# nv-dvl/nerfmatch

Measured on AMD Instinct MI355X. Metric: rays*samples/sec, higher is better.
Workload: dtype fp16x3 (fp16 MFMA on hi/lo-split fp32 operands, three products per fp32 product, fp32 accumulate; fp32 everywhere else)

## Files before the change

nerfmatch_amd/csrc/nerf_fwd_bf16.hip:

```cpp
#include "nerf_split_chain.h"

namespace {
using namespace nmbf;
using nmsample::HALF_PI_F32, nmsample::SCAN_TILE, nmsample::frustum, nmsample::ray_consts, nmsample::lift_var, nmsample::ipe_fast, nmsample::view_row_value;
using nmsample::alpha_of, nmsample::trans_factor, nmsample::sigmoid, nmsample::scan_before_barrier, nmsample::scan_after_barrier, nmsample::scan_carry;
using nmsample::first_max;
static_assert(TILE == SCAN_TILE, "the compositing scan of nerf_sample.h spans two wavefronts");

template <int PART, bool OWN>
__device__ __forceinline__ void tap_prefetch(Ctx& cx) {
  if constexpr (PART == 0) __builtin_amdgcn_s_barrier();
  const char* src = reinterpret_cast<const char*>(cx.tapw);
#pragma unroll
  for (int q = (PART == 0 ? 0 : 4); q < (PART == 0 ? 4 : 7); ++q) {
    const char* sp = src + q * 4096;
    const float* dp = q < 4 ? cx.tap_ring + q * 1024 : cx.tap_ipe + (q - 4) * 1024;
    const unsigned lds = (unsigned)__builtin_amdgcn_readfirstlane((int)(unsigned)(size_t)(const __attribute__((address_space(3))) float*)dp);
    if constexpr (OWN) {
      asm volatile("s_mov_b32 m0, %0\n\tglobal_load_lds_dwordx4 %1, off\n\tglobal_load_lds_dwordx4 %1, off offset:1024\n\t"
                   "global_load_lds_dwordx4 %1, off offset:2048\n\tglobal_load_lds_dwordx4 %1, off offset:3072"
                   :: "s"(lds), "v"(sp) : "memory");
      continue;
    }
    unsigned m0_saved;
    asm volatile("s_mov_b32 %0, m0\n\ts_mov_b32 m0, %1\n\tglobal_load_lds_dwordx4 %2, off\n\tglobal_load_lds_dwordx4 %2, off offset:1024\n\t"
                 "global_load_lds_dwordx4 %2, off offset:2048\n\tglobal_load_lds_dwordx4 %2, off offset:3072\n\ts_mov_b32 m0, %0"
                 : "=&s"(m0_saved) : "s"(lds), "v"(sp) : "memory");
  }
}

__device__ __forceinline__ void dpp_pairs8(float (&o)[8], const float (&x)[8], const float (&y)[8], bool eight) {
  if (eight)
    asm("s_nop 1\n"
        "v_add_f32_dpp %0, %8, %8 row_mirror row_mask:0xf bank_mask:0x3\n\tv_add_f32_dpp %1, %9, %9 row_mirror row_mask:0xf bank_mask:0x3\n\t"
        "v_add_f32_dpp %2, %10, %10 row_mirror row_mask:0xf bank_mask:0x3\n\tv_add_f32_dpp %3, %11, %11 row_mirror row_mask:0xf bank_mask:0x3\n\t"
        "v_add_f32_dpp %4, %12, %12 row_mirror row_mask:0xf bank_mask:0x3\n\tv_add_f32_dpp %5, %13, %13 row_mirror row_mask:0xf bank_mask:0x3\n\t"
        "v_add_f32_dpp %6, %14, %14 row_mirror row_mask:0xf bank_mask:0x3\n\tv_add_f32_dpp %7, %15, %15 row_mirror row_mask:0xf bank_mask:0x3\n\t"
        "v_add_f32_dpp %0, %16, %16 row_mirror row_mask:0xf bank_mask:0xc\n\tv_add_f32_dpp %1, %17, %17 row_mirror row_mask:0xf bank_mask:0xc\n\t"
        "v_add_f32_dpp %2, %18, %18 row_mirror row_mask:0xf bank_mask:0xc\n\tv_add_f32_dpp %3, %19, %19 row_mirror row_mask:0xf bank_mask:0xc\n\t"
        "v_add_f32_dpp %4, %20, %20 row_mirror row_mask:0xf bank_mask:0xc\n\tv_add_f32_dpp %5, %21, %21 row_mirror row_mask:0xf bank_mask:0xc\n\t"
        "v_add_f32_dpp %6, %22, %22 row_mirror row_mask:0xf bank_mask:0xc\n\tv_add_f32_dpp %7, %23, %23 row_mirror row_mask:0xf bank_mask:0xc"
        : "=&v"(o[0]), "=&v"(o[1]), "=&v"(o[2]), "=&v"(o[3]), "=&v"(o[4]), "=&v"(o[5]), "=&v"(o[6]), "=&v"(o[7])
        : "v"(x[0]), "v"(x[1]), "v"(x[2]), "v"(x[3]), "v"(x[4]), "v"(x[5]), "v"(x[6]), "v"(x[7]),
          "v"(y[0]), "v"(y[1]), "v"(y[2]), "v"(y[3]), "v"(y[4]), "v"(y[5]), "v"(y[6]), "v"(y[7]));
  else
    asm("s_nop 1\n"
        "v_add_f32_dpp %0, %8, %8 row_half_mirror row_mask:0xf bank_mask:0x5\n\tv_add_f32_dpp %1, %9, %9 row_half_mirror row_mask:0xf bank_mask:0x5\n\t"
        "v_add_f32_dpp %2, %10, %10 row_half_mirror row_mask:0xf bank_mask:0x5\n\tv_add_f32_dpp %3, %11, %11 row_half_mirror row_mask:0xf bank_mask:0x5\n\t"
        "v_add_f32_dpp %4, %12, %12 row_half_mirror row_mask:0xf bank_mask:0x5\n\tv_add_f32_dpp %5, %13, %13 row_half_mirror row_mask:0xf bank_mask:0x5\n\t"
        "v_add_f32_dpp %6, %14, %14 row_half_mirror row_mask:0xf bank_mask:0x5\n\tv_add_f32_dpp %7, %15, %15 row_half_mirror row_mask:0xf bank_mask:0x5\n\t"
        "v_add_f32_dpp %0, %16, %16 row_half_mirror row_mask:0xf bank_mask:0xa\n\tv_add_f32_dpp %1, %17, %17 row_half_mirror row_mask:0xf bank_mask:0xa\n\t"
        "v_add_f32_dpp %2, %18, %18 row_half_mirror row_mask:0xf bank_mask:0xa\n\tv_add_f32_dpp %3, %19, %19 row_half_mirror row_mask:0xf bank_mask:0xa\n\t"
        "v_add_f32_dpp %4, %20, %20 row_half_mirror row_mask:0xf bank_mask:0xa\n\tv_add_f32_dpp %5, %21, %21 row_half_mirror row_mask:0xf bank_mask:0xa\n\t"
        "v_add_f32_dpp %6, %22, %22 row_half_mirror row_mask:0xf bank_mask:0xa\n\tv_add_f32_dpp %7, %23, %23 row_half_mirror row_mask:0xf bank_mask:0xa"
        : "=&v"(o[0]), "=&v"(o[1]), "=&v"(o[2]), "=&v"(o[3]), "=&v"(o[4]), "=&v"(o[5]), "=&v"(o[6]), "=&v"(o[7])
        : "v"(x[0]), "v"(x[1]), "v"(x[2]), "v"(x[3]), "v"(x[4]), "v"(x[5]), "v"(x[6]), "v"(x[7]),
          "v"(y[0]), "v"(y[1]), "v"(y[2]), "v"(y[3]), "v"(y[4]), "v"(y[5]), "v"(y[6]), "v"(y[7]));
}
template <int XOR>
__device__ __forceinline__ void quad_add8(float (&v)[8]) {
  if (XOR == 1)
    asm("s_nop 1\n"
        "v_add_f32_dpp %0, %0, %0 quad_perm:[1,0,3,2] row_mask:0xf bank_mask:0xf\n\tv_add_f32_dpp %1, %1, %1 quad_perm:[1,0,3,2] row_mask:0xf bank_mask:0xf\n\t"
        "v_add_f32_dpp %2, %2, %2 quad_perm:[1,0,3,2] row_mask:0xf bank_mask:0xf\n\tv_add_f32_dpp %3, %3, %3 quad_perm:[1,0,3,2] row_mask:0xf bank_mask:0xf\n\t"
        "v_add_f32_dpp %4, %4, %4 quad_perm:[1,0,3,2] row_mask:0xf bank_mask:0xf\n\tv_add_f32_dpp %5, %5, %5 quad_perm:[1,0,3,2] row_mask:0xf bank_mask:0xf\n\t"
        "v_add_f32_dpp %6, %6, %6 quad_perm:[1,0,3,2] row_mask:0xf bank_mask:0xf\n\tv_add_f32_dpp %7, %7, %7 quad_perm:[1,0,3,2] row_mask:0xf bank_mask:0xf"
        : "+v"(v[0]), "+v"(v[1]), "+v"(v[2]), "+v"(v[3]), "+v"(v[4]), "+v"(v[5]), "+v"(v[6]), "+v"(v[7]));
  else
    asm("s_nop 1\n"
        "v_add_f32_dpp %0, %0, %0 quad_perm:[2,3,0,1] row_mask:0xf bank_mask:0xf\n\tv_add_f32_dpp %1, %1, %1 quad_perm:[2,3,0,1] row_mask:0xf bank_mask:0xf\n\t"
        "v_add_f32_dpp %2, %2, %2 quad_perm:[2,3,0,1] row_mask:0xf bank_mask:0xf\n\tv_add_f32_dpp %3, %3, %3 quad_perm:[2,3,0,1] row_mask:0xf bank_mask:0xf\n\t"
        "v_add_f32_dpp %4, %4, %4 quad_perm:[2,3,0,1] row_mask:0xf bank_mask:0xf\n\tv_add_f32_dpp %5, %5, %5 quad_perm:[2,3,0,1] row_mask:0xf bank_mask:0xf\n\t"
        "v_add_f32_dpp %6, %6, %6 quad_perm:[2,3,0,1] row_mask:0xf bank_mask:0xf\n\tv_add_f32_dpp %7, %7, %7 quad_perm:[2,3,0,1] row_mask:0xf bank_mask:0xf"
        : "+v"(v[0]), "+v"(v[1]), "+v"(v[2]), "+v"(v[3]), "+v"(v[4]), "+v"(v[5]), "+v"(v[6]), "+v"(v[7]));
}
__device__ __forceinline__ float reduce_scatter_step16(float x, float y) {
  const auto r = __builtin_amdgcn_permlane16_swap(__float_as_uint(x), __float_as_uint(y), false, false);
  return __uint_as_float(r[0]) + __uint_as_float(r[1]);
}
__device__ __forceinline__ f32x4 reduce_scatter_16pairs(const float (&s1)[64], int lane) {
  float s2[32];
#pragma unroll
  for (int b = 0; b < 4; ++b) {
    float o[8], x[8], y[8];
#pragma unroll
    for (int i = 0; i < 8; ++i) { x[i] = s1[8 * b + i]; y[i] = s1[32 + 8 * b + i]; }
    dpp_pairs8(o, x, y, true);
#pragma unroll
    for (int i = 0; i < 8; ++i) s2[8 * b + i] = o[i];
  }
  float s3[16];
#pragma unroll
  for (int b = 0; b < 2; ++b) {
    float o[8], x[8], y[8];
#pragma unroll
    for (int i = 0; i < 8; ++i) { x[i] = s2[8 * b + i]; y[i] = s2[16 + 8 * b + i]; }
    dpp_pairs8(o, x, y, false);
#pragma unroll
    for (int i = 0; i < 8; ++i) s3[8 * b + i] = o[i];
  }
  float lo8[8], hi8[8];
#pragma unroll
  for (int i = 0; i < 8; ++i) { lo8[i] = s3[i]; hi8[i] = s3[8 + i]; }
  quad_add8<2>(lo8); quad_add8<2>(hi8);
  float s4[8];
#pragma unroll
  for (int i = 0; i < 8; ++i) s4[i] = (lane & 2) ? hi8[i] : lo8[i];
  float t8[8] = {s4[0], s4[1], s4[2], s4[3], s4[4], s4[5], s4[6], s4[7]};
  quad_add8<1>(t8);
  return (lane & 1) ? f32x4{t8[4], t8[5], t8[6], t8[7]} : f32x4{t8[0], t8[1], t8[2], t8[3]};
}
__device__ __forceinline__ f32x4 reduce_scatter_32rows(float (&v)[128], int lane) {
  float s1[64];
#pragma unroll
  for (int i = 0; i < 64; ++i) s1[i] = reduce_scatter_step16(v[i], v[64 + i]);
  return reduce_scatter_16pairs(s1, lane);
}

#define NM_MLP_DONE_WAIT() __builtin_amdgcn_s_waitcnt(0x0070)
#define NM_EPI_BARRIER() asm volatile("s_waitcnt lgkmcnt(0)\n\ts_barrier" ::: "memory")
template <int P, bool TAP7 = true>
__device__ __forceinline__ void nerf_fwd_body(const NerfArgs& a) {
  constexpr bool DENS = P == 2 && !TAP7;
  __shared__ __attribute__((aligned(16))) float sm[LDS_TOTAL];
  float* const sm_small = sm + LDS_SMALL;
  float* const ring = sm + LDS_RING;
  float* const sm_ipe = sm + LDS_IPE;
  float* const sm_sigma = sm + LDS_SCR;
  float* const sm_rgb = sm_sigma + TILE;
  float* const sm_t0 = sm_rgb + 3 * TILE;
  float* const sm_t1 = sm_t0 + TILE;
  float* const sm_mean = sm_t1 + TILE;
  float* const sm_dn = sm_mean + 3 * TILE;
  float* const sm_w = sm_dn + TILE;
  float* const sm_misc = sm_w + TILE;
  float* const sm_part = sm_misc + 32;
  float* const sm_feat = sm + LDS_FEAT;
  float* const sm_ex = sm + LDS_EX;
  int* const sm_lray = reinterpret_cast<int*>(sm + LDS_LEFT);
  float* const sm_lT = sm + LDS_LEFT + TILE;
  unsigned* const sm_rng = reinterpret_cast<unsigned*>(sm + LDS_RNG);

  const int tid = threadIdx.x, lane = tid & 63, wave = tid >> 6, s = lane & 31, hi = lane >> 5;
  const bool tail_ok = a.left && !(a.tail_viol && *a.tail_viol != 0);
  const int S = a.S, R = a.R;
  const int Sa = tail_ok ? a.Sa : S;
  const int left = tail_ok ? 1 : 0;
  const int ntiles = tail_ok ? a.ntiles : a.ntiles_full;
  const int SP = Sa < TILE ? Sa : TILE;
  const int nr = TILE / SP;
  const int nchunks = (Sa + TILE - 1) / TILE;
  const bool need_rgb = !(a.flags & NM_NERF_SKIP_RGB);
  const bool feat_max = (a.flags & NM_NERF_FEAT_MAX) != 0;
  const bool need_tap = (a.feat != nullptr) || (a.sfeat != nullptr);
  const int tap = (a.tap < 0 || a.tap > 7) ? 7 : a.tap;
  const int nslots = need_rgb ? NSLOT_FULL : NSLOT_NORGB;
  const char* const blob_slots = a.blob + (size_t)SMALL_PAD * 4;

  for (int i = tid; i < SMALL / 4; i += 256) reinterpret_cast<f32x4*>(sm_small)[i] = reinterpret_cast<const f32x4*>(a.blob)[i];
  if constexpr (P == 2) {
#pragma unroll
    for (int k = 0; k < NRANGE; ++k) sm_rng[k * 256 + tid] = 0u;
  }

  int nleft = 0;
  int bid = blockIdx.x;
#pragma unroll 1
  for (;;) {
  bool lo_pass = false;
  if (left && (nleft > TILE - 4 || (bid >= ntiles && nleft > 0))) lo_pass = true;
  else if (bid >= ntiles) break;
  const int nent = lo_pass ? nleft : 0;
  TRACE(0);
  if (need_rgb && !lo_pass && tid < nr * 48) {
    const int r2 = tid / 48, f = tid % 48;
    const int ray2 = bid * nr + r2;
    const float* rq = a.rays + (size_t)(ray2 < R ? ray2 : R - 1) * 12 + 8;
    float v = view_row_value(f, rq[f % 3], a.app_row);
    if constexpr (P == 2) {
      v *= reinterpret_cast<const float*>(a.blob)[OFF_INSCALE + (f < 27 ? 1 : 2)];
      __hip_atomic_fetch_max(sm_rng + 9 * 256 + tid, __float_as_uint(fabsf(v)), __ATOMIC_RELAXED, __HIP_MEMORY_SCOPE_WORKGROUP);
    }
    sm_ex[tid] = v;
  }
  __syncthreads();
  TRACE(1);

  const int js = wave * 32 + s;
  const int rl = js / SP;
  const int ray = lo_pass ? (js < nent ? sm_lray[js] : R) : bid * nr + rl;
  const int rc = lo_pass ? sm_lray[js < nent ? js : 0] : (ray < R ? ray : R - 1);
  const float* rp = a.rays + (size_t)rc * 12;
  const float o0 = rp[0], o1 = rp[1], o2 = rp[2], d0 = rp[3], d1 = rp[4], d2 = rp[5], radius = rp[11];
  float dsq[3], nul[3], dnorm;
  ray_consts(rp + 3, dsq, nul, dnorm);

  float red_acc = 0.f;
  float carryT = 1.f;
  float best_w = -1.f;
  float feat_run = 0.f;

  const int nch = lo_pass ? 1 : nchunks;
  for (int chunk = 0; chunk < nch; ++chunk) {
    const int sidx = lo_pass ? Sa : chunk * TILE + (js % SP);
    const float t0 = a.t[(size_t)rc * (S + 1) + sidx];
    const float t1 = a.t[(size_t)rc * (S + 1) + sidx + 1];
// ... 34 lines not shown
    if constexpr (is_split<P>()) {
      ring_open_wait<P>(cx);
    } else {
      ring_acquire<P>(blob_slots, 0, nslots, ring, wave, lane);
    }
    load_half<P>(cx.opA, ring, lane, 0);
    if constexpr (P == 1) load_half<1>(cx.opB, ring, lane, 1);
    const float* ipe_src = sm_ipe + wave * (XS * 2 * 64 * 4) + lane * 4;

    auto composite_weights = [&]() __attribute__((always_inline)) {
      const int tid2 = launder(threadIdx.x), lane2 = tid2 & 63, wave2 = tid2 >> 6;
      float alpha = 0.f, incl = 1.f;
      if (tid2 < TILE) {
        alpha = alpha_of(sm_sigma[tid2], (sm_t1[tid2] - sm_t0[tid2]) * sm_dn[tid2]);
        incl = scan_before_barrier(trans_factor(alpha), lane2, wave2, SP, sm_misc);
      }
      NM_EPI_BARRIER();
      if (tid2 < TILE) {
        const float excl = scan_after_barrier(incl, lane2, wave2, SP, sm_misc, carryT);
        sm_w[tid2] = alpha * excl;
        const int r2 = tid2 / SP, ray2 = bid * nr + r2;
        if (left && chunk == nchunks - 1 && ray2 < R && tid2 % SP == SP - 1) {
          sm_lray[nleft + r2] = ray2;
          sm_lT[nleft + r2] = excl * trans_factor(alpha);
        }
      }
      if (nchunks > 1) carryT = scan_carry(carryT, sm_misc);
    };
    auto composite_sums = [&]() __attribute__((always_inline)) {
      const int tid2 = launder(threadIdx.x);
      if (tid2 < TILE) {
        const float wgt = sm_w[tid2];
        const int r2 = tid2 / SP, ray2 = bid * nr + r2;
        if (ray2 < R) {
          const int s2 = chunk * TILE + tid2 % SP;
          a.weights[(size_t)ray2 * S + s2] = wgt;
          if (left && chunk == nchunks - 1) {
            for (int k = Sa + 1 + tid2 % SP; k < S; k += SP) a.weights[(size_t)ray2 * S + k] = 0.f;
          }
          if (a.raw && !NM_TRACE) {
            f32x4 rv = {sm_rgb[tid2], sm_rgb[TILE + tid2], sm_rgb[2 * TILE + tid2], sm_sigma[tid2]};
            *reinterpret_cast<f32x4*>(a.raw + ((size_t)ray2 * S + s2) * 4) = rv;
          }
        }
        float pq[8] = {wgt, wgt * sm_rgb[tid2], wgt * sm_rgb[TILE + tid2], wgt * sm_rgb[2 * TILE + tid2],
                       wgt * (0.5f * (sm_t0[tid2] + sm_t1[tid2])), wgt * sm_mean[tid2], wgt * sm_mean[TILE + tid2],
                       wgt * sm_mean[2 * TILE + tid2]};
        nm_half_sum_dpp8(pq);
        if ((tid2 & 31) == 16) {
          *reinterpret_cast<f32x4*>(sm_part + (tid2 >> 5) * 8) = f32x4{pq[0], pq[1], pq[2], pq[3]};
          *reinterpret_cast<f32x4*>(sm_part + (tid2 >> 5) * 8 + 4) = f32x4{pq[4], pq[5], pq[6], pq[7]};
        }
      }
    };
    auto pick_best = [&]() __attribute__((always_inline)) {
      const int tid2 = launder(threadIdx.x);
      if (tid2 < 8 * nr) {
        const int q = tid2 & 7, r2 = tid2 >> 3;
        const float* wv = sm_w + r2 * SP;
        int bi;
        const bool better = first_max(wv, SP, best_w, bi);
        if (q == 0) sm_misc[8 + r2] = better ? __int_as_float(r2 * SP + bi) : __int_as_float(-1);
        if (q >= 5 && better) red_acc = sm_mean[(q - 5) * TILE + r2 * SP + bi];
      }
    };
    auto tap7_early = [&](Ctx& c) __attribute__((always_inline)) {
      const int t2 = launder(threadIdx.x), jl = (t2 >> 6) * 32 + (t2 & 31), hl = (t2 >> 5) & 1;
      const float sigma_raw = (c.sig_part + nm_shfl_xor32(c.sig_part)) + sm_small[OFF_MISC];
      if (hl == 0) sm_sigma[jl] = sigma_raw;
      NM_EPI_BARRIER();
      composite_weights();
      NM_EPI_BARRIER();
      if (feat_max) {
        pick_best();
        NM_EPI_BARRIER();
      }
      const float desc = sm_small[OFF_DESCALE + 7];
      const float wj = sm_w[jl] * desc;
      const int best = feat_max ? __float_as_int(sm_misc[8 + jl / SP]) : -2;
      const float mult = feat_max ? (jl == best ? desc : 0.f) : wj;
      const float* bl = sm_small + OFF_BIAS + 7 * 256 + 4 * hl;
      const float s7 = sm_small[OFF_SCALE + 7];
      float s1[64];
#pragma unroll
      for (int cq = 0; cq < HS; ++cq) {
        const f32x4 b0 = *reinterpret_cast<const f32x4*>(bl + (cq >> 2) * 32 + 8 * (cq & 3));
        const f32x4 b1 = *reinterpret_cast<const f32x4*>(bl + (4 + (cq >> 2)) * 32 + 8 * (cq & 3));
#pragma unroll
        for (int e = 0; e < 4; ++e) {
          const float x = mult * __builtin_fmaxf(__builtin_fmaf(c.hv[4 * cq + e], s7, b0[e]), 0.f);
          const float y = mult * __builtin_fmaxf(__builtin_fmaf(c.hv[64 + 4 * cq + e], s7, b1[e]), 0.f);
          s1[4 * cq + e] = reduce_scatter_step16(x, y);
        }
      }
      const f32x4 sum4 = reduce_scatter_16pairs(s1, jl);
      const int r = jl & 31;
      float* prow = sm_feat + (jl >> 5) * 256 + 4 * hl;
      *reinterpret_cast<f32x4*>(prow + (r >> 2) * 32 + 16 * ((r >> 1) & 1) + 8 * (r & 1)) = sum4;
    };
    const Tap7InRegisters<decltype(tap7_early)> tap7{early, tap7_early};
    f32x16 acc[8];
    ipe_steps<P, true>(acc, cx, ipe_src);
    finish_layer<P>(acc, 0, cx);
    TRACE(3);
#pragma unroll 1
    for (int l = 1; l < 8; ++l) {
      layer_pass<P, DENS>(acc, l, cx, ipe_src, tap7);
      TRACE(3 + l);
    }
    float c_r = 0.f, c_g = 0.f, c_b = 0.f;
    if (!need_rgb) {
      if (cx.tap == 7) dump_tap(7, cx);
      NM_MLP_DONE_WAIT();
      if (cx.tap_pref) tap_prefetch<0, owns_m0<P>()>(cx);
      alpha_head(cx);
      if (cx.tap_pref) tap_prefetch<1, owns_m0<P>()>(cx);
    } else {
      const int hh = launder(lane) >> 5;
      const float* exr = sm_ex + launder(rl) * 48 + 8 * hh;
      f32x16 av[4];
      if constexpr (DENS) {
        views_hidden<P, true>(av, cx);
        dens_close(cx);
      } else views_hidden<P>(av, cx);
      fold_range<P>(cx, 7);
      bf16x8 exh[VS], exl[VS];
#pragma unroll
      for (int e = 0; e < VS; ++e) {
        float v8[8];
        if (!lo_pass) {
          const f32x4 e0 = *reinterpret_cast<const f32x4*>(exr + 16 * e), e1 = *reinterpret_cast<const f32x4*>(exr + 16 * e + 4);
          v8[0] = e0[0]; v8[1] = e0[1]; v8[2] = e0[2]; v8[3] = e0[3]; v8[4] = e1[0]; v8[5] = e1[1]; v8[6] = e1[2]; v8[7] = e1[3];
        } else {
          const float* rq = a.rays + (size_t)launder(rc) * 12 + 8;
          const float vd0 = rq[0], vd1 = rq[1], vd2 = rq[2];
#pragma unroll
          for (int i = 0; i < 8; ++i) {
            const int f = 16 * e + 8 * hh + i;
            const int ax = f % 3;
            float v = view_row_value(f, ax == 0 ? vd0 : ax == 1 ? vd1 : vd2, a.app_row);
            if constexpr (P == 2) v *= sm_small[OFF_INSCALE + (f < 27 ? 1 : 2)];
            v8[i] = v;
          }
        }
        if constexpr (is_split<P>()) split8_p<P>(v8, exh[e], exl[e]);
        else exh[e] = exl[e] = pack8_f16(v8);
      }
      views_extras<P>(av, cx, exh, exl, a.app_row == nullptr);
      TRACE(11);
      NM_MLP_DONE_WAIT();
      if (cx.tap_pref) tap_prefetch<0, owns_m0<P>()>(cx);
      const float* bv = sm_small + OFF_BVIEWS + 4 * hh;
      const float* wr = sm_small + OFF_WRGB + 4 * hh;
      float pr = 0.f, pg = 0.f, pb = 0.f;
#pragma unroll
      for (int ob = 0; ob < 4; ++ob) {
#pragma unroll
        for (int q = 0; q < 4; ++q) {
          const f32x4 b4 = *reinterpret_cast<const f32x4*>(bv + ob * 32 + 8 * q);
          const f32x4 wr4 = *reinterpret_cast<const f32x4*>(wr + ob * 32 + 8 * q);
          const f32x4 wg4 = *reinterpret_cast<const f32x4*>(wr + 128 + ob * 32 + 8 * q);
          const f32x4 wb4 = *reinterpret_cast<const f32x4*>(wr + 256 + ob * 32 + 8 * q);
#pragma unroll
          for (int e = 0; e < 4; ++e) {
            const float hv = __builtin_fmaxf(acc_read(av[ob][4 * q + e]) + b4[e], 0.f);
            pr = NM_FMA(hv, wr4[e], pr);
            pg = NM_FMA(hv, wg4[e], pg);
            pb = NM_FMA(hv, wb4[e], pb);
          }
        }
      }
      pr = (pr + nm_shfl_xor32(pr)) + sm_small[OFF_MISC + 1];
      pg = (pg + nm_shfl_xor32(pg)) + sm_small[OFF_MISC + 2];
      pb = (pb + nm_shfl_xor32(pb)) + sm_small[OFF_MISC + 3];
      c_r = sigmoid(pr);
      c_g = sigmoid(pg);
      c_b = sigmoid(pb);
      if (cx.tap_pref) tap_prefetch<1, owns_m0<P>()>(cx);
    }
    const float sigma_raw = (cx.sig_part + nm_shfl_xor32(cx.sig_part)) + sm_small[OFF_MISC];
    TRACE(12);
    {
      const int jsw = launder(js);
      if ((launder(lane) >> 5) == 0) {
        sm_sigma[jsw] = sigma_raw;
        sm_rgb[jsw] = c_r; sm_rgb[TILE + jsw] = c_g; sm_rgb[2 * TILE + jsw] = c_b;
      }
    }
    NM_EPI_BARRIER();
    TRACE(13);
    const int tid2 = launder(threadIdx.x), lane2 = tid2 & 63, wave2 = tid2 >> 6;

    if (lo_pass) {
      if (tid2 < nent) {
        const int ray2 = sm_lray[tid2];
        const float wgt = alpha_of(sm_sigma[tid2], (sm_t1[tid2] - sm_t0[tid2]) * sm_dn[tid2]) * sm_lT[tid2];
        sm_w[tid2] = wgt;
        a.weights[(size_t)ray2 * S + Sa] = wgt;
        if (a.acc) atomicAdd(a.acc + ray2, wgt);
        if (a.rgb && need_rgb) {
#pragma unroll
          for (int c = 0; c < 3; ++c) atomicAdd(a.rgb + (size_t)ray2 * 3 + c, a.white_bg ? wgt * sm_rgb[c * TILE + tid2] - wgt : wgt * sm_rgb[c * TILE + tid2]);
        }
        if (a.depth) atomicAdd(a.depth + ray2, wgt * (0.5f * (sm_t0[tid2] + sm_t1[tid2])));
        if (a.pts) {
#pragma unroll
          for (int c = 0; c < 3; ++c) atomicAdd(a.pts + (size_t)ray2 * 3 + c, wgt * sm_mean[c * TILE + tid2]);
        }
      }
      __syncthreads();
      if (need_tap) {
        const int jl = launder(js), hl = launder(lane) >> 5;
        const f32x4* tw = reinterpret_cast<const f32x4*>(a.ws) + ((size_t)blockIdx.x * 4 + wave2) * 32 * 64 + lane2;
        if (jl < nent) {
          const int ray2 = sm_lray[jl];
          const float desc = sm_small[OFF_DESCALE + tap];
          const float wj = sm_w[jl] * desc;
#pragma unroll 4
          for (int ks = 0; ks < HS; ++ks) {
            const f32x4 ta = tw[(2 * ks) * 64], tb = tw[(2 * ks + 1) * 64];
            const int n0 = (ks >> 1) * 32 + 16 * (ks & 1) + 4 * hl;
            if (a.sfeat) {
              float* dsf = a.sfeat + ((size_t)ray2 * S + Sa) * 256 + n0;
              *reinterpret_cast<f32x4*>(dsf) = ta * desc;
              *reinterpret_cast<f32x4*>(dsf + 8) = tb * desc;
            }
            if (a.feat) {
              float* df = a.feat + (size_t)ray2 * 256 + n0;
#pragma unroll
              for (int e = 0; e < 4; ++e) {
                atomicAdd(df + e, wj * ta[e]);
                atomicAdd(df + 8 + e, wj * tb[e]);
              }
            }
          }
        }
      }
      __syncthreads();
      break;
    }

    if (!early) composite_weights();
    composite_sums();
    NM_EPI_BARRIER();

    if (tid2 < 8 * nr) {
      const int q = tid2 & 7, r2 = tid2 >> 3;
      if (!feat_max || q < 5) {
        float sum = 0.f;
        for (int hw = r2 * (SP / 32); hw < (r2 + 1) * (SP / 32); ++hw) sum += sm_part[hw * 8 + q];
        red_acc += sum;
      }
    }
    if (feat_max && !early) {
      pick_best();
      NM_EPI_BARRIER();
    }

    TRACE(14);
    if (need_tap && !early) {
      const int jl = launder(js), hl = launder(lane) >> 5;
// ... 163 lines not shown
```

nerfmatch_amd/csrc/nerf_split_chain.h:

```cpp
#pragma once
#include "nerf_bf16_common.h"

namespace nmbf {

template <int P> constexpr bool is_bf16() { return P == 0 || P == 3 || P == 4; }
template <int P> constexpr bool has_gates() { return P == 4; }
typedef _Float16 f16x8 __attribute__((ext_vector_type(8)));
typedef _Float16 f16x2 __attribute__((ext_vector_type(2)));
template <int P>
__device__ __forceinline__ f32x16 mfma_p(const bf16x8& a, const bf16x8& b, const f32x16& c) {
  if constexpr (is_bf16<P>()) return MFMA_BF16(a, b, c);
  else return __builtin_amdgcn_mfma_f32_32x32x16_f16(__builtin_bit_cast(f16x8, a), __builtin_bit_cast(f16x8, b), c, 0, 0, 0);
}
template <int P> constexpr bool is_split() { return P != 1; }
template <int P> constexpr int slot_bytes() { return is_split<P>() ? SLOT_BYTES : SLOT_BYTES / 2; }
template <int P> constexpr int slot_floats() { return slot_bytes<P>() / 4; }
template <int P> constexpr int ring_slots() { return is_split<P>() ? NRING : 2 * NRING; }
template <int P> constexpr int ring_ahead() { return is_split<P>() ? 4 : 6; }
constexpr float F16_MAX = 65504.0f;
__device__ __forceinline__ void split8_f16(const float (&v)[8], bf16x8& hi, bf16x8& lo) {
  f16x8 h8, l8;
#pragma unroll
  for (int i = 0; i < 8; ++i) {
    const float c = __builtin_amdgcn_fmed3f(v[i], -F16_MAX, F16_MAX);
// ... 417 lines not shown
  }
};
constexpr int take_n(int s) { return s == 0 ? 4 : s == 1 ? 2 : s <= 4 ? 3 : s == 10 ? 2 : 5; }
constexpr int take_before(int s) {
  int n = 0;
  for (int k = 0; k < s; ++k) n += take_n(k);
  return n;
}
constexpr int TAKE_HIDDEN = take_before(12);
__device__ __forceinline__ const float* unit0_bias(const Ctx& cx, int l) { return cx.sm_small + OFF_BIAS + l * 256 + 4 * cx.hi; }
template <int P>
struct AccTake {
  const f32x16 (&acc)[8];
  Ctx& cx;
  int l;
  __device__ __forceinline__ void prefetch() {}
  __device__ __forceinline__ void operator()(int j) {
#pragma unroll
    for (int k = 0; k < 8; ++k) {
      const int i = 8 * j + k;
      if (i < 64) cx.hv[i] = acc_read(acc[i >> 4][i & 15]);
    }
  }
  __device__ __forceinline__ void seq(int) {}
  template <bool EVEN> __device__ __forceinline__ void step8(int t) {
    if (t < 12) return;
    const int s = t - 12;
#pragma unroll
    for (int k = 0; k < take_n(s); ++k) {
      const int i = take_before(s) + k;
      cx.hv[i] = acc_read(acc[i >> 4][i & 15]);
    }
    if (s == 10) {
      const float* bl = unit0_bias(cx, l);
      cx.hb0 = *reinterpret_cast<const f32x4*>(bl); cx.hb1 = *reinterpret_cast<const f32x4*>(bl + 8);
    }
  }
};
template <int P, bool DENS = false>
__device__ __forceinline__ UnitWork<P, DENS> unit_work(int u, int lo, Ctx& cx, Unit& out) {
  return UnitWork<P, DENS>{cx, out, u, lo, lo < 8 ? 0.f : (!is_bf16<P>() ? -F16_MAX : -__builtin_inff()), {}, {}, cx.sc, {}, 0.f, 0.f, {}, {}, {}, {}};
}

template <int P>
__device__ __forceinline__ void finish_layer(const f32x16 (&acc)[8], int l, Ctx& cx) {
  if constexpr (is_split<P>()) {
#pragma unroll
    for (int i = TAKE_HIDDEN; i < 64; ++i) cx.hv[i] = acc_read(acc[i >> 4][i & 15]);
  }
#pragma unroll
  for (int ob = 4; ob < 8; ++ob)
#pragma unroll
    for (int r = 0; r < 16; ++r) cx.hv[ob * 16 + r] = acc_read(acc[ob][r]);
  if constexpr (P == 2)
    cx.sc = __builtin_bit_cast(float, __builtin_amdgcn_readfirstlane(__builtin_bit_cast(int, cx.sm_small[OFF_SCALE + l])));
  UnitWork<P> w = unit_work<P>(0, l, cx, cx.xn);
  if constexpr (P == 2) {
    const float* bl = unit0_bias(cx, l) + 16;
    cx.nb0 = *reinterpret_cast<const f32x4*>(bl); cx.nb1 = *reinterpret_cast<const f32x4*>(bl + 8);
  }
  if constexpr (is_split<P>()) {
    w.b0 = cx.hb0; w.b1 = cx.hb1;
#pragma unroll
    for (int j = 0; j < 4; ++j) w.relu(j);
#pragma unroll
    for (int p = 0; p < 4; ++p) {
      w.hi(p);
      if constexpr (is_bf16<P>()) w.rem(p);
    }
    if constexpr (!is_bf16<P>()) {
#pragma unroll
      for (int p = 0; p < 4; ++p) w.rem(p);
    }
#pragma unroll
    for (int p = 0; p < 4; ++p) w.lo(p);
    w.gates();
  } else {
    w.prefetch();
#pragma unroll
    for (int j = 0; j < 12; ++j) w(j);
  }
}

__device__ __forceinline__ void alpha_head(Ctx& cx) {
  const float* bl = cx.sm_small + OFF_BIAS + 7 * 256 + 4 * cx.hi;
  const float* wa = cx.sm_small + OFF_WALPHA + 4 * cx.hi;
  const float s7 = cx.sm_small[OFF_SCALE + 7];
  float p0 = 0.f, p1 = 0.f, p2 = 0.f, p3 = 0.f;
#pragma unroll
  for (int ob = 0; ob < 8; ++ob)
#pragma unroll
    for (int q = 0; q < 4; ++q) {
      const f32x4 b = *reinterpret_cast<const f32x4*>(bl + ob * 32 + 8 * q);
      const f32x4 w4v = *reinterpret_cast<const f32x4*>(wa + ob * 32 + 8 * q);
      p0 = NM_FMA(__builtin_fmaxf(__builtin_fmaf(cx.hv[ob * 16 + 4 * q + 0], s7, b[0]), 0.f), w4v[0], p0);
      p1 = NM_FMA(__builtin_fmaxf(__builtin_fmaf(cx.hv[ob * 16 + 4 * q + 1], s7, b[1]), 0.f), w4v[1], p1);
      p2 = NM_FMA(__builtin_fmaxf(__builtin_fmaf(cx.hv[ob * 16 + 4 * q + 2], s7, b[2]), 0.f), w4v[2], p2);
      p3 = NM_FMA(__builtin_fmaxf(__builtin_fmaf(cx.hv[ob * 16 + 4 * q + 3], s7, b[3]), 0.f), w4v[3], p3);
    }
  cx.sig_part = (p0 + p1) + (p2 + p3);
}

__device__ __forceinline__ void dens_open(Ctx& cx) {
  const float* bl = cx.sm_small + OFF_BIAS + 7 * 256 + 4 * cx.hi;
  const float* wa = cx.sm_small + OFF_WALPHA + 4 * cx.hi;
  const f32x4 b0 = *reinterpret_cast<const f32x4*>(bl), b1 = *reinterpret_cast<const f32x4*>(bl + 8);
  const f32x4 w0 = *reinterpret_cast<const f32x4*>(wa), w1 = *reinterpret_cast<const f32x4*>(wa + 8);
  float v[8];
#pragma unroll
  for (int j = 0; j < 4; ++j) {
    v[j] = __builtin_fmaxf(__builtin_fmaf(cx.hv[j], cx.sc, b0[j]), 0.f);
    v[4 + j] = __builtin_fmaxf(__builtin_fmaf(cx.hv[4 + j], cx.sc, b1[j]), 0.f);
  }
#pragma unroll
  for (int j = 0; j < 4; ++j) cx.dp[j] = NM_FMA(v[j], w0[j], 0.f);
  cx.dp[0] = NM_FMA(v[4], w1[0], cx.dp[0]);
#pragma unroll
  for (int j = 0; j < 3; ++j) { cx.dv[j] = v[5 + j]; cx.dw[j] = w1[1 + j]; }
}
struct DensTail {
  Ctx& cx;
  __device__ __forceinline__ void seq(int c) {
    if (c == 1) {
#pragma unroll
      for (int j = 0; j < 3; ++j) UnitWork<2, true>::dens_fma(cx.dp[1 + j], cx.dv[j], cx.dw[j]);
    }
  }
};
__device__ __forceinline__ void dens_close(Ctx& cx) { cx.sig_part = (cx.dp[0] + cx.dp[1]) + (cx.dp[2] + cx.dp[3]); }

__device__ __forceinline__ void dump_tap(int lo, Ctx& cx) {
  const float* bl = cx.sm_small + OFF_BIAS + lo * 256 + 4 * cx.hi;
  const float sl = cx.sm_small[OFF_SCALE + lo];
  auto* tp = (__attribute__((address_space(1))) f32x4*)cx.tapw;
#pragma unroll
  for (int ob = 0; ob < 8; ++ob) {
    f32x4 v[4];
#pragma unroll
    for (int q = 0; q < 4; ++q) {
      const f32x4 b = *reinterpret_cast<const f32x4*>(bl + ob * 32 + 8 * q);
#pragma unroll
      for (int e = 0; e < 4; ++e) v[q][e] = __builtin_fmaxf(__builtin_fmaf(cx.hv[ob * 16 + 4 * q + e], sl, b[e]), 0.f);
    }
#pragma unroll
    for (int q = 0; q < 4; ++q) tp[q * 64] = v[q];
    tp += 256;
    pin(tp);
  }
}

__device__ __forceinline__ bf16x8 load_op1(const float* slot, int lane, int blk) {
  return __builtin_bit_cast(bf16x8, (reinterpret_cast<const u32x4*>(slot) + lane)[blk * 64]);
}
#define NM_SB __builtin_amdgcn_sched_barrier(0)
template <bool FIRST, bool ACQ, class Work>
__device__ __forceinline__ void slot_step8_one(f32x16 (&acc)[8], Ctx& cx, const bf16x8& x, Work work) {
  const f32x16 zero = {0.f, 0.f, 0.f, 0.f, 0.f, 0.f, 0.f, 0.f, 0.f, 0.f, 0.f, 0.f, 0.f, 0.f, 0.f, 0.f};
  const int g = cx.g;
  const OpHalf A = cx.opA, B = cx.opB;
  const float* nxt = ring_slot<1>(cx.ring, g + 1);
  acc[0] = mfma_p<1>(A.h[0], x, FIRST ? zero : acc[0]); NM_SB;
  if constexpr (ACQ) ring_acquire_pair(cx.blob_slots, g, cx.ring, cx.wave, cx.lane);
  NM_SB;
  acc[1] = mfma_p<1>(A.h[1], x, FIRST ? zero : acc[1]); NM_SB;
  cx.opA.h[0] = load_op1(nxt, cx.lane, 0); cx.opA.h[1] = load_op1(nxt, cx.lane, 1); work.prefetch(); NM_SB;
  acc[2] = mfma_p<1>(A.h[2], x, FIRST ? zero : acc[2]); NM_SB;
  cx.opA.h[2] = load_op1(nxt, cx.lane, 2); cx.opA.h[3] = load_op1(nxt, cx.lane, 3); NM_SB;
  acc[3] = mfma_p<1>(A.h[3], x, FIRST ? zero : acc[3]); NM_SB;
  cx.opB.h[0] = load_op1(nxt, cx.lane, 4); cx.opB.h[1] = load_op1(nxt, cx.lane, 5); NM_SB;
  acc[4] = mfma_p<1>(B.h[0], x, FIRST ? zero : acc[4]); NM_SB;
  cx.opB.h[2] = load_op1(nxt, cx.lane, 6); cx.opB.h[3] = load_op1(nxt, cx.lane, 7); NM_SB;
  acc[5] = mfma_p<1>(B.h[1], x, FIRST ? zero : acc[5]); NM_SB;
  work(0); work(1); NM_SB;
  acc[6] = mfma_p<1>(B.h[2], x, FIRST ? zero : acc[6]); NM_SB;
  work(2); work(3); work(4); NM_SB;
  acc[7] = mfma_p<1>(B.h[3], x, FIRST ? zero : acc[7]); NM_SB;
  work(5); work(6); work(7); NM_SB;
  cx.g = g + 1;
}

template <int P>
__device__ __forceinline__ void load_pair(OpHalf& d, const float* slot, int lane, int p, int o) {
  const u32x4* s4 = reinterpret_cast<const u32x4*>(slot) + lane;
  d.h[o] = __builtin_bit_cast(bf16x8, s4[((4 * p + o) * 2 + 0) * 64]);
  d.l[o] = __builtin_bit_cast(bf16x8, s4[((4 * p + o) * 2 + 1) * 64]);
}
template <int P, bool FIRST>
__device__ __forceinline__ f32x16 mfma_k(int k, const OpHalf& a, const bf16x8& xh, const bf16x8& xl, const f32x16& c) {
  const f32x16 zero = {0.f, 0.f, 0.f, 0.f, 0.f, 0.f, 0.f, 0.f, 0.f, 0.f, 0.f, 0.f, 0.f, 0.f, 0.f, 0.f};
  if (k < 4) return mfma_p<P>(a.h[k], xh, FIRST ? zero : c);
  if (k < 8) return mfma_p<P>(a.h[k & 3], xl, c);
  return mfma_p<P>(a.l[k & 3], xh, c);
}

template <int P, bool FIRST, bool EVEN, bool RQE = false, class Work>
__device__ __forceinline__ void slot_step8(f32x16 (&acc)[8], Ctx& cx, const bf16x8& xh, const bf16x8& xl, Work work) {
  if constexpr (P == 1) {
    slot_step8_one<FIRST, EVEN>(acc, cx, xh, work);
    return;
  }
  const int g = cx.g;
  const OpHalf A = cx.opA;
  OpHalf B;
  const float* cur = cx.ring + (g & (NRING - 1)) * SLOT_FLOATS;
  const float* nxt = cx.ring + ((g + 1) & (NRING - 1)) * SLOT_FLOATS;
#pragma unroll
  for (int k = 0; k < 12; ++k) {
    acc[k & 3] = mfma_k<P, FIRST>(k, A, xh, xl, acc[k & 3]);
    __builtin_amdgcn_sched_barrier(0);
    if (k < 4) load_pair<P>(B, cur, cx.lane, 1, k);
    if constexpr (EVEN && !RQE) {
      if (k == 2 || k == 3) ring_arm<P>(cx, k - 2);
      if (k >= 4) ring_request<P>(cx, g, k - 4);
    }
    if constexpr (EVEN && RQE) {
      if (k == 4 || k == 5) ring_request<P>(cx, g, k + 2);
    }
    if constexpr (!EVEN && RQE) {
      if (k == 5) ring_arm<P>(cx, 0);
    }
    work.template step8<EVEN>(k);
    __builtin_amdgcn_sched_barrier(0);
  }
  if constexpr (!EVEN) {
    ring_acquire_two();
    __builtin_amdgcn_sched_barrier(0);
  }
#pragma unroll
  for (int k = 0; k < 12; ++k) {
    acc[4 + (k & 3)] = mfma_k<P, FIRST>(k, B, xh, xl, acc[4 + (k & 3)]);
    __builtin_amdgcn_sched_barrier(0);
// ... 98 lines not shown
#pragma unroll
    for (int sl = 0; sl < HS / 2; ++sl) {
      const Unit x0 = cx.xn;
      Unit u1;
      const bf16x8 x0h = __builtin_bit_cast(bf16x8, x0.h), x0l = __builtin_bit_cast(bf16x8, x0.l);
      if (sl == 0) slot_step4x2<P, true, true>(av, cx, x0h, x0l, u1, unit_work<P, DENS>(1, 7, cx, u1), unit_work<P, DENS>(2, 7, cx, cx.xn));
      else if (sl + 1 == HS / 2) {
        if constexpr (DENS) slot_step4x2<P, false, false>(av, cx, x0h, x0l, u1, unit_work<P, DENS>(2 * sl + 1, 7, cx, u1), DensTail{cx});
        else slot_step4x2<P, false, false>(av, cx, x0h, x0l, u1, unit_work<P>(2 * sl + 1, 7, cx, u1), NoWork{});
      } else if (sl & 1) slot_step4x2<P, false, false>(av, cx, x0h, x0l, u1, unit_work<P, DENS>(2 * sl + 1, 7, cx, u1), unit_work<P, DENS>(2 * sl + 2, 7, cx, cx.xn));
      else slot_step4x2<P, false, true>(av, cx, x0h, x0l, u1, unit_work<P, DENS>(2 * sl + 1, 7, cx, u1), unit_work<P, DENS>(2 * sl + 2, 7, cx, cx.xn));
    }
  } else {
#pragma unroll
    for (int ks = 0; ks < HS; ks += 2) {
      {
        const Unit xc = cx.xn;
        if (ks == 0) slot_step4<P, true, true>(av, cx, __builtin_bit_cast(bf16x8, xc.h), __builtin_bit_cast(bf16x8, xc.l), unit_work<P>(ks + 1, 7, cx, cx.xn));
        else slot_step4<P, false, true>(av, cx, __builtin_bit_cast(bf16x8, xc.h), __builtin_bit_cast(bf16x8, xc.l), unit_work<P>(ks + 1, 7, cx, cx.xn));
      }
      {
        const Unit xc = cx.xn;
        if (ks + 2 < HS) slot_step4<P, false, false>(av, cx, __builtin_bit_cast(bf16x8, xc.h), __builtin_bit_cast(bf16x8, xc.l), unit_work<P>(ks + 2, 7, cx, cx.xn));
        else slot_step4<P, false, false>(av, cx, __builtin_bit_cast(bf16x8, xc.h), __builtin_bit_cast(bf16x8, xc.l), NoWork{});
      }
    }
  }
}
template <int P>
__device__ __forceinline__ void views_extras(f32x16 (&av)[4], Ctx& cx, const bf16x8 (&eh)[VS], const bf16x8 (&el)[VS], bool no_app) {
  if constexpr (is_split<P>()) {
    Unit u1;
    u1.h = __builtin_bit_cast(u32x4, eh[1]); u1.l = __builtin_bit_cast(u32x4, el[1]);
    slot_step4x2<P, false, true>(av, cx, eh[0], el[0], u1, NoWork{}, NoWork{});
    if (!no_app) slot_step4<P, false, false>(av, cx, eh[2], el[2], NoWork{});
  } else {
    slot_step4<P, false, true>(av, cx, eh[0], el[0], NoWork{});
    slot_step4<P, false, false>(av, cx, eh[1], el[1], NoWork{});
    if (!no_app) slot_step4<P, false, true>(av, cx, eh[2], el[2], NoWork{});
  }
}

template <int P, bool FIRST>
__device__ __forceinline__ void ipe_steps(f32x16 (&acc)[8], Ctx& cx, const float* ipe_src, int l = FIRST ? 0 : 5) {
  auto operand = [&](int m, bf16x8& ph, bf16x8& pl) {
    ph = __builtin_bit_cast(bf16x8, *reinterpret_cast<const u32x4*>(ipe_src + (is_split<P>() ? (m * 2 + 0) : m) * 256));
    pl = ph;
    if constexpr (is_split<P>()) pl = __builtin_bit_cast(bf16x8, *reinterpret_cast<const u32x4*>(ipe_src + (m * 2 + 1) * 256));
  };
  if constexpr (P == 2) {
    bf16x8 ph, pl, qh, ql;
    operand(0, ph, pl);
#pragma unroll
    for (int m = 0; m < XS; m += 2) {
      if (m == 0) slot_step8<P, FIRST, true>(acc, cx, ph, pl, IpeFetch<17>{ipe_src, m + 1, qh, ql});
      else slot_step8<P, false, true, true>(acc, cx, ph, pl, IpeFetch<6>{ipe_src, m + 1, qh, ql});
      if (m + 2 == XS) slot_step8<P, false, false>(acc, cx, qh, ql, AccTake<P>{acc, cx, l});
      else slot_step8<P, false, false, true>(acc, cx, qh, ql, IpeFetch<4>{ipe_src, m + 2, ph, pl});
    }
    return;
  }
#pragma unroll
  for (int m = 0; m < XS; m += 2) {
    bf16x8 ph, pl;
    operand(m, ph, pl);
    if (m == 0) slot_step8<P, FIRST, true>(acc, cx, ph, pl, NoWork{});
    else slot_step8<P, false, true>(acc, cx, ph, pl, NoWork{});
    operand(m + 1, ph, pl);
    if (m + 2 == XS) slot_step8<P, false, false>(acc, cx, ph, pl, AccTake<P>{acc, cx, l});
    else slot_step8<P, false, false>(acc, cx, ph, pl, NoWork{});
  }
}

struct Tap7Workspace {
  static constexpr bool on = false;
  __device__ __forceinline__ void fn(Ctx&) const {}
};
template <class F>
struct Tap7InRegisters {
  bool on;
  F fn;
};

template <int P, bool DENS = false, class Tap7 = Tap7Workspace>
__device__ __forceinline__ void layer_pass(f32x16 (&acc)[8], int l, Ctx& cx, const float* ipe_src, const Tap7& tap7 = Tap7()) {
  if (l - 1 == cx.tap) dump_tap(l - 1, cx);
#pragma unroll
  for (int ks = 0; ks < HS; ks += 2) {
    {
      const Unit xc = cx.xn;
      if (ks == 0) slot_step8<P, true, true>(acc, cx, __builtin_bit_cast(bf16x8, xc.h), __builtin_bit_cast(bf16x8, xc.l), unit_work<P>(ks + 1, l - 1, cx, cx.xn));
      else slot_step8<P, false, true, request_early<P>()>(acc, cx, __builtin_bit_cast(bf16x8, xc.h), __builtin_bit_cast(bf16x8, xc.l), unit_work<P>(ks + 1, l - 1, cx, cx.xn));
    }
    {
      const Unit xc = cx.xn;
      if (ks + 2 < HS) slot_step8<P, false, false, request_early<P>()>(acc, cx, __builtin_bit_cast(bf16x8, xc.h), __builtin_bit_cast(bf16x8, xc.l), unit_work<P>(ks + 2, l - 1, cx, cx.xn));
      else slot_step8<P, false, false>(acc, cx, __builtin_bit_cast(bf16x8, xc.h), __builtin_bit_cast(bf16x8, xc.l), AccTake<P>{acc, cx, l});
    }
  }
  fold_range<P>(cx, l - 1);
  if constexpr (has_gates<P>()) {
    cx.gptr[(l - 1) * 256] = u32x4{cx.gbits[0], cx.gbits[1], cx.gbits[2], cx.gbits[3]};
    cx.gbits[0] = cx.gbits[1] = cx.gbits[2] = cx.gbits[3] = 0u;
  }
  if (l == 5) ipe_steps<P, false>(acc, cx, ipe_src);
  finish_layer<P>(acc, l, cx);
  if (l == 7) {
    if (cx.rgb) {
      if (cx.tap == 7 && !tap7.on) dump_tap(7, cx);
      if constexpr (DENS) dens_open(cx);
      else alpha_head(cx);
      if (tap7.on) tap7.fn(cx);
    }
  }
}

}
```

Baseline: 397.8 million.

## Software-pipeline LDS loads one step ahead in heads and spread tap DMA

Adds a helper that loads the next LDS weight/bias group while computing the current one, with sched barriers to keep that ordering. It is applied to the alpha head, tap dump, tap7 reduction and RGB head for split variants. It also breaks the tap-prefetch global-to-LDS DMA into pieces issued one per RGB-head iteration with scalar base addressing, instead of two bursts. This is meant to hide LDS latency and overlap the DMA with ALU work, at the cost of extra registers and a rigid hand-set schedule.

Result: slower. 391.0 million (-1.7%).

```diff
diff --git a/nerfmatch_amd/csrc/nerf_fwd_bf16.hip b/nerfmatch_amd/csrc/nerf_fwd_bf16.hip
--- a/nerfmatch_amd/csrc/nerf_fwd_bf16.hip
+++ b/nerfmatch_amd/csrc/nerf_fwd_bf16.hip
@@ -27,6 +27,34 @@
                  "global_load_lds_dwordx4 %2, off offset:2048\n\tglobal_load_lds_dwordx4 %2, off offset:3072\n\ts_mov_b32 m0, %0"
                  : "=&s"(m0_saved) : "s"(lds), "v"(sp) : "memory");
   }
+}
+
+__device__ __forceinline__ void tap_ring_free() { __builtin_amdgcn_s_barrier(); }
+__device__ __forceinline__ const char* tap_base(const Ctx& cx) {
+  const size_t p = reinterpret_cast<size_t>(cx.tapw) - cx.dma_voff;
+  const unsigned lo = (unsigned)__builtin_amdgcn_readfirstlane((int)(unsigned)p), hi = (unsigned)__builtin_amdgcn_readfirstlane((int)(unsigned)(p >> 32));
+  return reinterpret_cast<const char*>(((size_t)hi << 32) | lo);
+}
+__device__ __forceinline__ void tap_piece(const Ctx& cx, const char* base, int j) {
+  const int q = j >> 2;
+  const char* sp = base + q * 4096;
+  if ((j & 3) == 0) {
+    const float* dp = q < 4 ? cx.tap_ring + q * 1024 : cx.tap_ipe + (q - 4) * 1024;
+    const unsigned lds = (unsigned)__builtin_amdgcn_readfirstlane((int)(unsigned)(size_t)(const __attribute__((address_space(3))) float*)dp);
+    asm volatile("s_mov_b32 m0, %0" :: "s"(lds) : "memory");
+  }
+  switch (j & 3) {
+    case 0: asm volatile("global_load_lds_dwordx4 %0, %1" :: "v"(cx.dma_voff), "s"(sp) : "memory"); break;
+    case 1: asm volatile("global_load_lds_dwordx4 %0, %1 offset:1024" :: "v"(cx.dma_voff), "s"(sp) : "memory"); break;
+    case 2: asm volatile("global_load_lds_dwordx4 %0, %1 offset:2048" :: "v"(cx.dma_voff), "s"(sp) : "memory"); break;
+    default: asm volatile("global_load_lds_dwordx4 %0, %1 offset:3072" :: "v"(cx.dma_voff), "s"(sp) : "memory"); break;
+  }
+}
+__device__ __forceinline__ void tap_spread(const Ctx& cx, const char* base, int g) {
+  if (g < 12) {
+    tap_piece(cx, base, 2 * g);
+    tap_piece(cx, base, 2 * g + 1);
+  } else tap_piece(cx, base, 12 + g);
 }
 
 __device__ __forceinline__ void dpp_pairs8(float (&o)[8], const float (&x)[8], const float (&y)[8], bool eight) {
@@ -122,6 +150,7 @@
 template <int P, bool TAP7 = true>
 __device__ __forceinline__ void nerf_fwd_body(const NerfArgs& a) {
   constexpr bool DENS = P == 2 && !TAP7;
+  constexpr bool AHEAD = is_split<P>();
   __shared__ __attribute__((aligned(16))) float sm[LDS_TOTAL];
   float* const sm_small = sm + LDS_SMALL;
   float* const ring = sm + LDS_RING;
@@ -322,17 +351,30 @@
       const float* bl = sm_small + OFF_BIAS + 7 * 256 + 4 * hl;
       const float s7 = sm_small[OFF_SCALE + 7];
       float s1[64];
-#pragma unroll
-      for (int cq = 0; cq < HS; ++cq) {
-        const f32x4 b0 = *reinterpret_cast<const f32x4*>(bl + (cq >> 2) * 32 + 8 * (cq & 3));
-        const f32x4 b1 = *reinterpret_cast<const f32x4*>(bl + (4 + (cq >> 2)) * 32 + 8 * (cq & 3));
-#pragma unroll
-        for (int e = 0; e < 4; ++e) {
-          const float x = mult * __builtin_fmaxf(__builtin_fmaf(c.hv[4 * cq + e], s7, b0[e]), 0.f);
-          const float y = mult * __builtin_fmaxf(__builtin_fmaf(c.hv[64 + 4 * cq + e], s7, b1[e]), 0.f);
-          s1[4 * cq + e] = reduce_scatter_step16(x, y);
-        }
-      }
+      if constexpr (!AHEAD) {
+#pragma unroll
+        for (int cq = 0; cq < HS; ++cq) {
+          const f32x4 b0 = *reinterpret_cast<const f32x4*>(bl + (cq >> 2) * 32 + 8 * (cq & 3));
+          const f32x4 b1 = *reinterpret_cast<const f32x4*>(bl + (4 + (cq >> 2)) * 32 + 8 * (cq & 3));
+#pragma unroll
+          for (int e = 0; e < 4; ++e) {
+            const float x = mult * __builtin_fmaxf(__builtin_fmaf(c.hv[4 * cq + e], s7, b0[e]), 0.f);
+            const float y = mult * __builtin_fmaxf(__builtin_fmaf(c.hv[64 + 4 * cq + e], s7, b1[e]), 0.f);
+            s1[4 * cq + e] = reduce_scatter_step16(x, y);
+          }
+        }
+      } else lds_one_ahead<HS>(
+          [&](int cq) {
+            return LdsSet<2>{{*reinterpret_cast<const f32x4*>(bl + 8 * cq), *reinterpret_cast<const f32x4*>(bl + 128 + 8 * cq)}};
+          },
+          [&](int cq, const LdsSet<2>& r) {
+#pragma unroll
+            for (int e = 0; e < 4; ++e) {
+              const float x = mult * __builtin_fmaxf(__builtin_fmaf(c.hv[4 * cq + e], s7, r.v[0][e]), 0.f);
+              const float y = mult * __builtin_fmaxf(__builtin_fmaf(c.hv[64 + 4 * cq + e], s7, r.v[1][e]), 0.f);
+              s1[4 * cq + e] = reduce_scatter_step16(x, y);
+            }
+          });
       const f32x4 sum4 = reduce_scatter_16pairs(s1, jl);
       const int r = jl & 31;
       float* prow = sm_feat + (jl >> 5) * 256 + 4 * hl;
@@ -345,15 +387,15 @@
     TRACE(3);
 #pragma unroll 1
     for (int l = 1; l < 8; ++l) {
-      layer_pass<P, DENS>(acc, l, cx, ipe_src, tap7);
+      layer_pass<P, DENS, AHEAD>(acc, l, cx, ipe_src, tap7);
       TRACE(3 + l);
     }
     float c_r = 0.f, c_g = 0.f, c_b = 0.f;
     if (!need_rgb) {
-      if (cx.tap == 7) dump_tap(7, cx);
+      if (cx.tap == 7) dump_tap<AHEAD>(7, cx);
       NM_MLP_DONE_WAIT();
       if (cx.tap_pref) tap_prefetch<0, owns_m0<P>()>(cx);
-      alpha_head(cx);
+      alpha_head<AHEAD>(cx);
       if (cx.tap_pref) tap_prefetch<1, owns_m0<P>()>(cx);
     } else {
       const int hh = launder(lane) >> 5;
@@ -389,26 +431,53 @@
       views_extras<P>(av, cx, exh, exl, a.app_row == nullptr);
       TRACE(11);
       NM_MLP_DONE_WAIT();
-      if (cx.tap_pref) tap_prefetch<0, owns_m0<P>()>(cx);
+      constexpr bool SPREAD = AHEAD && owns_m0<P>();
+      if (cx.tap_pref) {
+        if constexpr (SPREAD) tap_ring_free();
+        else tap_prefetch<0, owns_m0<P>()>(cx);
+      }
       const float* bv = sm_small + OFF_BVIEWS + 4 * hh;
       const float* wr = sm_small + OFF_WRGB + 4 * hh;
       float pr = 0.f, pg = 0.f, pb = 0.f;
-#pragma unroll
-      for (int ob = 0; ob < 4; ++ob) {
-#pragma unroll
-        for (int q = 0; q < 4; ++q) {
-          const f32x4 b4 = *reinterpret_cast<const f32x4*>(bv + ob * 32 + 8 * q);
-          const f32x4 wr4 = *reinterpret_cast<const f32x4*>(wr + ob * 32 + 8 * q);
-          const f32x4 wg4 = *reinterpret_cast<const f32x4*>(wr + 128 + ob * 32 + 8 * q);
-          const f32x4 wb4 = *reinterpret_cast<const f32x4*>(wr + 256 + ob * 32 + 8 * q);
-#pragma unroll
-          for (int e = 0; e < 4; ++e) {
-            const float hv = __builtin_fmaxf(acc_read(av[ob][4 * q + e]) + b4[e], 0.f);
-            pr = NM_FMA(hv, wr4[e], pr);
-            pg = NM_FMA(hv, wg4[e], pg);
-            pb = NM_FMA(hv, wb4[e], pb);
+      if constexpr (!AHEAD) {
+#pragma unroll
+        for (int ob = 0; ob < 4; ++ob) {
+#pragma unroll
+          for (int q = 0; q < 4; ++q) {
+            const f32x4 b4 = *reinterpret_cast<const f32x4*>(bv + ob * 32 + 8 * q);
+            const f32x4 wr4 = *reinterpret_cast<const f32x4*>(wr + ob * 32 + 8 * q);
+            const f32x4 wg4 = *reinterpret_cast<const f32x4*>(wr + 128 + ob * 32 + 8 * q);
+            const f32x4 wb4 = *reinterpret_cast<const f32x4*>(wr + 256 + ob * 32 + 8 * q);
+#pragma unroll
+            for (int e = 0; e < 4; ++e) {
+              const float hv = __builtin_fmaxf(acc_read(av[ob][4 * q + e]) + b4[e], 0.f);
+              pr = NM_FMA(hv, wr4[e], pr);
+              pg = NM_FMA(hv, wg4[e], pg);
+              pb = NM_FMA(hv, wb4[e], pb);
+            }
           }
         }
+      } else {
+        const char* const tapb = SPREAD ? tap_base(cx) : nullptr;
+        auto head = [&](auto pieces) __attribute__((always_inline)) {
+          lds_one_ahead<16>(
+              [&](int g) {
+                return LdsSet<4>{{*reinterpret_cast<const f32x4*>(bv + 8 * g), *reinterpret_cast<const f32x4*>(wr + 8 * g),
+                                  *reinterpret_cast<const f32x4*>(wr + 128 + 8 * g), *reinterpret_cast<const f32x4*>(wr + 256 + 8 * g)}};
+              },
+              [&](int g, const LdsSet<4>& r) {
+#pragma unroll
+                for (int e = 0; e < 4; ++e) {
+                  const float hv = __builtin_fmaxf(acc_read(av[g >> 2][4 * (g & 3) + e]) + r.v[0][e], 0.f);
+                  pr = NM_FMA(hv, r.v[1][e], pr);
+                  pg = NM_FMA(hv, r.v[2][e], pg);
+                  pb = NM_FMA(hv, r.v[3][e], pb);
+                }
+                if constexpr (decltype(pieces)::value) tap_spread(cx, tapb, g);
+              });
+        };
+        if (SPREAD && cx.tap_pref) head(std::true_type{});
+        else head(std::false_type{});
       }
       pr = (pr + nm_shfl_xor32(pr)) + sm_small[OFF_MISC + 1];
       pg = (pg + nm_shfl_xor32(pg)) + sm_small[OFF_MISC + 2];
@@ -416,7 +485,9 @@
       c_r = sigmoid(pr);
       c_g = sigmoid(pg);
       c_b = sigmoid(pb);
-      if (cx.tap_pref) tap_prefetch<1, owns_m0<P>()>(cx);
+      if constexpr (!SPREAD) {
+        if (cx.tap_pref) tap_prefetch<1, owns_m0<P>()>(cx);
+      }
     }
     const float sigma_raw = (cx.sig_part + nm_shfl_xor32(cx.sig_part)) + sm_small[OFF_MISC];
     TRACE(12);
diff --git a/nerfmatch_amd/csrc/nerf_split_chain.h b/nerfmatch_amd/csrc/nerf_split_chain.h
--- a/nerfmatch_amd/csrc/nerf_split_chain.h
+++ b/nerfmatch_amd/csrc/nerf_split_chain.h
@@ -523,22 +523,51 @@
   }
 }
 
+template <int K>
+struct LdsSet {
+  f32x4 v[K];
+};
+template <int N, class Load, class Use>
+__device__ __forceinline__ void lds_one_ahead(Load load, Use use) {
+  auto cur = load(0);
+#pragma unroll
+  for (int g = 0; g < N; ++g) {
+    auto nxt = cur;
+    if (g + 1 < N) nxt = load(g + 1);
+    __builtin_amdgcn_sched_barrier(0);
+    use(g, cur);
+    __builtin_amdgcn_sched_barrier(0);
+    cur = nxt;
+  }
+}
+
+template <bool AHEAD = false>
 __device__ __forceinline__ void alpha_head(Ctx& cx) {
   const float* bl = cx.sm_small + OFF_BIAS + 7 * 256 + 4 * cx.hi;
   const float* wa = cx.sm_small + OFF_WALPHA + 4 * cx.hi;
   const float s7 = cx.sm_small[OFF_SCALE + 7];
   float p0 = 0.f, p1 = 0.f, p2 = 0.f, p3 = 0.f;
-#pragma unroll
-  for (int ob = 0; ob < 8; ++ob)
-#pragma unroll
-    for (int q = 0; q < 4; ++q) {
-      const f32x4 b = *reinterpret_cast<const f32x4*>(bl + ob * 32 + 8 * q);
-      const f32x4 w4v = *reinterpret_cast<const f32x4*>(wa + ob * 32 + 8 * q);
-      p0 = NM_FMA(__builtin_fmaxf(__builtin_fmaf(cx.hv[ob * 16 + 4 * q + 0], s7, b[0]), 0.f), w4v[0], p0);
-      p1 = NM_FMA(__builtin_fmaxf(__builtin_fmaf(cx.hv[ob * 16 + 4 * q + 1], s7, b[1]), 0.f), w4v[1], p1);
-      p2 = NM_FMA(__builtin_fmaxf(__builtin_fmaf(cx.hv[ob * 16 + 4 * q + 2], s7, b[2]), 0.f), w4v[2], p2);
-      p3 = NM_FMA(__builtin_fmaxf(__builtin_fmaf(cx.hv[ob * 16 + 4 * q + 3], s7, b[3]), 0.f), w4v[3], p3);
-    }
+  if constexpr (!AHEAD) {
+#pragma unroll
+    for (int ob = 0; ob < 8; ++ob)
+#pragma unroll
+      for (int q = 0; q < 4; ++q) {
+        const f32x4 b = *reinterpret_cast<const f32x4*>(bl + ob * 32 + 8 * q);
+        const f32x4 w4v = *reinterpret_cast<const f32x4*>(wa + ob * 32 + 8 * q);
+        p0 = NM_FMA(__builtin_fmaxf(__builtin_fmaf(cx.hv[ob * 16 + 4 * q + 0], s7, b[0]), 0.f), w4v[0], p0);
+        p1 = NM_FMA(__builtin_fmaxf(__builtin_fmaf(cx.hv[ob * 16 + 4 * q + 1], s7, b[1]), 0.f), w4v[1], p1);
+        p2 = NM_FMA(__builtin_fmaxf(__builtin_fmaf(cx.hv[ob * 16 + 4 * q + 2], s7, b[2]), 0.f), w4v[2], p2);
+        p3 = NM_FMA(__builtin_fmaxf(__builtin_fmaf(cx.hv[ob * 16 + 4 * q + 3], s7, b[3]), 0.f), w4v[3], p3);
+      }
+  } else lds_one_ahead<32>(
+      [&](int g) { return LdsSet<2>{{*reinterpret_cast<const f32x4*>(bl + g * 8), *reinterpret_cast<const f32x4*>(wa + g * 8)}}; },
+      [&](int g, const LdsSet<2>& r) {
+        const f32x4 b = r.v[0], w4v = r.v[1];
+        p0 = NM_FMA(__builtin_fmaxf(__builtin_fmaf(cx.hv[4 * g + 0], s7, b[0]), 0.f), w4v[0], p0);
+        p1 = NM_FMA(__builtin_fmaxf(__builtin_fmaf(cx.hv[4 * g + 1], s7, b[1]), 0.f), w4v[1], p1);
+        p2 = NM_FMA(__builtin_fmaxf(__builtin_fmaf(cx.hv[4 * g + 2], s7, b[2]), 0.f), w4v[2], p2);
+        p3 = NM_FMA(__builtin_fmaxf(__builtin_fmaf(cx.hv[4 * g + 3], s7, b[3]), 0.f), w4v[3], p3);
+      });
   cx.sig_part = (p0 + p1) + (p2 + p3);
 }
 
@@ -570,24 +599,47 @@
 };
 __device__ __forceinline__ void dens_close(Ctx& cx) { cx.sig_part = (cx.dp[0] + cx.dp[1]) + (cx.dp[2] + cx.dp[3]); }
 
+template <bool AHEAD = false>
 __device__ __forceinline__ void dump_tap(int lo, Ctx& cx) {
   const float* bl = cx.sm_small + OFF_BIAS + lo * 256 + 4 * cx.hi;
   const float sl = cx.sm_small[OFF_SCALE + lo];
   auto* tp = (__attribute__((address_space(1))) f32x4*)cx.tapw;
-#pragma unroll
-  for (int ob = 0; ob < 8; ++ob) {
-    f32x4 v[4];
-#pragma unroll
-    for (int q = 0; q < 4; ++q) {
-      const f32x4 b = *reinterpret_cast<const f32x4*>(bl + ob * 32 + 8 * q);
-#pragma unroll
-      for (int e = 0; e < 4; ++e) v[q][e] = __builtin_fmaxf(__builtin_fmaf(cx.hv[ob * 16 + 4 * q + e], sl, b[e]), 0.f);
-    }
-#pragma unroll
-    for (int q = 0; q < 4; ++q) tp[q * 64] = v[q];
-    tp += 256;
-    pin(tp);
-  }
+  if constexpr (!AHEAD) {
+#pragma unroll
+    for (int ob = 0; ob < 8; ++ob) {
+      f32x4 v[4];
+#pragma unroll
+      for (int q = 0; q < 4; ++q) {
+        const f32x4 b = *reinterpret_cast<const f32x4*>(bl + ob * 32 + 8 * q);
+#pragma unroll
+        for (int e = 0; e < 4; ++e) v[q][e] = __builtin_fmaxf(__builtin_fmaf(cx.hv[ob * 16 + 4 * q + e], sl, b[e]), 0.f);
+      }
+#pragma unroll
+      for (int q = 0; q < 4; ++q) tp[q * 64] = v[q];
+      tp += 256;
+      pin(tp);
+    }
+    return;
+  }
+  lds_one_ahead<8>(
+      [&](int ob) {
+        LdsSet<4> r;
+#pragma unroll
+        for (int q = 0; q < 4; ++q) r.v[q] = *reinterpret_cast<const f32x4*>(bl + ob * 32 + 8 * q);
+        return r;
+      },
+      [&](int ob, const LdsSet<4>& r) {
+        f32x4 v[4];
+#pragma unroll
+        for (int q = 0; q < 4; ++q) {
+#pragma unroll
+          for (int e = 0; e < 4; ++e) v[q][e] = __builtin_fmaxf(__builtin_fmaf(cx.hv[ob * 16 + 4 * q + e], sl, r.v[q][e]), 0.f);
+          tp[q * 64] = v[q];
+          __builtin_amdgcn_sched_barrier(0);
+        }
+        tp += 256;
+        pin(tp);
+      });
 }
 
 __device__ __forceinline__ bf16x8 load_op1(const float* slot, int lane, int blk) {
@@ -852,9 +904,9 @@
   F fn;
 };
 
-template <int P, bool DENS = false, class Tap7 = Tap7Workspace>
+template <int P, bool DENS = false, bool AHEAD = false, class Tap7 = Tap7Workspace>
 __device__ __forceinline__ void layer_pass(f32x16 (&acc)[8], int l, Ctx& cx, const float* ipe_src, const Tap7& tap7 = Tap7()) {
-  if (l - 1 == cx.tap) dump_tap(l - 1, cx);
+  if (l - 1 == cx.tap) dump_tap<AHEAD>(l - 1, cx);
 #pragma unroll
   for (int ks = 0; ks < HS; ks += 2) {
     {
@@ -877,9 +929,9 @@
   finish_layer<P>(acc, l, cx);
   if (l == 7) {
     if (cx.rgb) {
-      if (cx.tap == 7 && !tap7.on) dump_tap(7, cx);
+      if (cx.tap == 7 && !tap7.on) dump_tap<AHEAD>(7, cx);
       if constexpr (DENS) dens_open(cx);
-      else alpha_head(cx);
+      else alpha_head<AHEAD>(cx);
       if (tap7.on) tap7.fn(cx);
     }
   }
```
